# zyansheep/shadow

Measured on AMD Instinct MI355X. Metric: APSP routing build (s) @10k nodes; packets routed/sec per sim round, lower is better.
Workload: dtype u64+f32; 1 GPU; C3 APSP routing build: 10k-node undirected ring+chords graph, mean degree 8, latency U[1,100] ms (integer us), loss 0 w.p. 0.8 else U(0,0.02); all nodes used; source rows sharded across ranks (each rank keeps its row block; the optional RCCL all-gather of the blocks is timed separately in apsp_detail.allgather_ms); nodes=10000, arcs=79996, parallelism=rows1

## Files before the change

### shadow_amd/csrc/sg_internal.h

```cpp
#pragma once

#include <hip/hip_runtime.h>

#include <cstdint>
#include <cstdio>
#include <new>
#include <stdexcept>
#include <string>
#include <atomic>
#include <deque>
#include <memory>
#include <vector>

#include "../../include/shadow_gpu.h"

namespace sg {

struct Error : std::runtime_error {
  int32_t code;
  uint32_t row, col;
  Error(int32_t c, const std::string& m, uint32_t r = 0, uint32_t k = 0)
      : std::runtime_error(m), code(c), row(r), col(k) {}
};

// ... 315 lines not shown

constexpr int SSSP_DIAG_WORDS = 16;
constexpr int SSSP_POP_CLASSES = 6;
constexpr int SSSP_POP_WORDS = 3 * SSSP_POP_CLASSES + 2;
struct SsspLdsLaunch {
  const uint32_t* d_used = nullptr;
  uint32_t n_used = 0, row_begin = 0, row_end = 0;
  bool ident = false;
  uint64_t* out_lat = nullptr;
  float* out_loss = nullptr;
  uint32_t* sat_row = nullptr;
  uint32_t delta = 0;
  unsigned long long* work = nullptr;
  unsigned long long* diag = nullptr;
  unsigned long long* pops = nullptr;
  const uint32_t* blk_rows = nullptr;
  uint32_t n_blk = 0;
  const uint32_t* ub_row = nullptr;
  const uint32_t* ub_w = nullptr;
  const uint32_t* plan_ctl = nullptr;
  int plan_ph = 0;
  uint32_t* plan_ctr = nullptr;
  uint32_t* done = nullptr;
  const SsspChainDesc* chain = nullptr;
};
void launch_sssp_lds(sg_ctx* ctx, const sg_net* net, const SsspLdsLaunch& l);

void ensure_csc(sg_ctx* ctx, sg_net* net);
void ensure_links(sg_ctx* ctx, sg_net* net);
std::string node_name(const sg_net* net, uint32_t idx);
void launch_zero2(sg_ctx* ctx, uint32_t* a, uint32_t na, uint32_t* b, uint32_t nb);

constexpr int WORK_SHARDS = 64;
void shortest_paths_slab(sg_ctx* ctx, sg_net* net, const uint32_t* d_used, uint32_t n_used, uint32_t row_begin,
                         uint32_t row_end, uint64_t* out_lat, float* out_loss);
void run_wide(sg_ctx* ctx, sg_net* net, const uint32_t* d_used, uint32_t n_used, const std::vector<uint32_t>& rows,
              uint32_t out_row0, uint64_t* out_lat, float* out_loss);

struct SsspDevPlan {
  int n_phase = 0;
  uint32_t* list = nullptr;
  uint32_t* ub_row = nullptr;
  uint32_t* ub_w = nullptr;
  uint32_t* ctl = nullptr;
  uint32_t* ctr = nullptr;
  const SsspChainDesc* chain = nullptr;
  bool landmarks = false;
  unsigned rows_grid = 0;
  bool bounds_deferred = false;
  const uint32_t* rel = nullptr;
  const uint8_t* phase_of = nullptr;
};
constexpr int SSSP_PHASES_MAX = 6;
SsspDevPlan sssp_device_plan(sg_ctx* ctx, sg_net* net, const uint32_t* d_used, uint32_t n_used, uint32_t row_begin,
                             uint32_t row_end, int n_phase, int kb, bool exact, int hops, uint32_t n_land,
                             uint32_t* zero_rows = nullptr, uint32_t* zero_rows2 = nullptr, bool chain = false,
                             bool chain_exact = false, bool defer_bounds = false);
void sssp_plan_bounds_side(sg_ctx* ctx, const sg_net* net, const SsspDevPlan& p, const uint32_t* d_used,
                           uint32_t row_begin, uint32_t row_end, int kb, bool exact, int hops);
const SsspChainDesc* sssp_plain_rel(sg_ctx* ctx, const sg_net* net, const uint32_t* d_used, uint32_t row_begin,
                                    uint32_t row_end, uint32_t* zero_rows, uint32_t* claim, uint32_t* zero_ctr,
                                    bool chain_exact);
void sssp_landmark_bounds(sg_ctx* ctx, const SsspDevPlan& p, uint32_t n_used, uint32_t row_begin,
                          const uint64_t* out_lat, const uint32_t* sat_row, int kb);

}
// ... 1 lines not shown
```

### shadow_amd/csrc/sg_routing.hip

```cpp
#include <algorithm>
#include <cstring>
#include <string>
#include <vector>

#include "sg_device.h"
#include "sg_internal.h"
#include "sg_knobs.h"

namespace sg {

__global__ void k_self_check(const uint32_t* __restrict__ used, uint32_t n_used,
                             const uint32_t* __restrict__ self_cnt,
                             unsigned long long* __restrict__ first) {
  for (uint32_t j = blockIdx.x * blockDim.x + threadIdx.x; j < n_used; j += gridDim.x * blockDim.x) {
    uint32_t c = self_cnt[used[j]];
    if (c != 1) atomicMin(first, ((unsigned long long)j << 1) | (c > 1 ? 1ull : 0ull));
  }
}

__global__ void __launch_bounds__(1024) k_build_finish(const uint32_t* __restrict__ sat, uint32_t rows,
                                                       const uint32_t* __restrict__ used, uint32_t n_used,
                                                       const uint32_t* __restrict__ self_cnt, uint32_t* __restrict__ ret,
                                                       int count_flags) {
  constexpr int G = 8;
// ... 288 lines not shown
  bool chain;
  bool overlap;
};
static LdsKnobs lds_knobs(const sg_ctx* ctx, const sg_net* net, uint32_t n_used, uint32_t rows) {
  LdsKnobs k;
  k.delta = (uint32_t)std::min(4294967295.0, std::max(1.0, knob_double("SG_APSP_DELTA", 4294967295.0)));
  k.diag = knob_int("SG_SSSP_DIAG", 0) != 0;
  const int seeds_env = knob_int("SG_SSSP_SEEDS", 1);
  const int flag_env = knob_int("SG_SSSP_FLAGGED", -1);
  const bool few_rows = rows < 6u * (uint32_t)std::max(1, ctx->n_cu);
  k.flagged = seeds_env != 0 && (flag_env == 1 || (flag_env < 0 && rows < n_used && !few_rows));
  k.phased = !k.flagged && seeds_env != 0 && (seeds_env == 2 || rows >= 8u * (uint32_t)ctx->n_cu);
  const bool chain = !knob_off("SG_SSSP_CHAIN") && !net->directed && !k.flagged;
  const uint32_t per_cu = rows / std::max(1, ctx->n_cu);
  k.n_phase = knob_int("SG_SSSP_PHASES", per_cu >= 16 && !chain ? 3 : 2, 2, SSSP_PHASES_MAX);
  k.kb = knob_int("SG_SSSP_BOUNDS", 2, 1, SSSP_KB_MAX);
  k.exact = knob_int("SG_SSSP_EXACT", 1) != 0 && n_used == net->n_nodes;
  k.hops = knob_int("SG_SSSP_HOPS", 3, 1, 3);
  const int land_env = knob_int("SG_SSSP_LANDMARKS", 0);
  k.n_land = net->directed || land_env <= 0 ? 0u : (uint32_t)land_env;
  k.chain = chain;
  k.overlap = build_fused();
  return k;
}

static void print_sssp_diag(sg_ctx* ctx, const sg_net* net, const unsigned long long* diag, uint32_t n_diag,
                            uint32_t delta) {
  constexpr int DW = SSSP_DIAG_WORDS;
  std::vector<unsigned long long> h((size_t)n_diag * DW);
  copy_to_host(ctx, h.data(), diag, h.size() * 8);
  double a[DW] = {};
  double setup = 0;
  double cn[2] = {0, 0}, cs[2] = {0, 0}, cq[2] = {0, 0};
  for (uint32_t r = 0; r < n_diag; r++) {
    for (int k = 0; k < DW; k++) a[k] += (double)h[(size_t)r * DW + k];
    const unsigned long long w3 = h[(size_t)r * DW + 3];
    setup += (double)(w3 >> 24);
    a[3] -= (double)(w3 >> 22 << 22);
    if (h[(size_t)r * DW] == 0) continue;
    const int c = (int)((w3 >> 22) & 1);
    cn[c] += 1;
    cs[c] += (double)(w3 >> 24);
    cq[c] += (double)h[(size_t)r * DW];
  }
  for (int c = 0; c < 2; c++)
    fprintf(stderr, "[sssp] %s rows: %.0f, mean setup %.0f cyc, mean search %.0f cyc\n", c ? "chained" : "unchained",
            cn[c], cs[c] / std::max(1.0, cn[c]), cq[c] / std::max(1.0, cn[c]));
  fprintf(stderr, "[sssp] mean setup (init + bound rows) %.0f cyc of the search\n", setup / n_diag);
  fprintf(stderr, "[sssp] setup parts: bound-row listing and load issue %.0f, LDS pass %.0f, barrier %.0f, first load "
          "round %.0f, later rounds and closing barrier %.0f cyc\n", a[9] / n_diag, a[8] / n_diag, a[10] / n_diag,
          a[11] / n_diag, a[12] / n_diag);
  fprintf(stderr, "[sssp] per-wave cycles summed over a row's 16 waves: claim+wait %.0f, pop %.0f, steps %.0f "
          "(per pop: %.0f, %.0f)\n", a[5] / n_diag, a[6] / n_diag, a[7] / n_diag, a[6] / std::max(1.0, a[2]),
          a[7] / std::max(1.0, a[2]));
  fprintf(stderr, "[sssp] delta %u ns, %u rows: mean search %.0f cyc, output %.0f cyc, %.1f wave pops, %.1f buckets, "
          "%.0f relaxations (%.2f x arcs)\n", delta, n_diag, a[0] / n_diag, a[1] / n_diag, a[2] / n_diag,
          a[3] / n_diag, a[4] / n_diag, a[4] / n_diag / std::max(1u, net->n_arcs));
}

static void shortest_paths_lds(sg_ctx* ctx, sg_net* net, const uint32_t* d_used, uint32_t n_used, uint32_t row_begin,
                               uint32_t row_end, uint64_t* out_lat, float* out_loss) {
  hipStream_t st = ctx->stream;
  const uint32_t rows = row_end - row_begin;
  const LdsKnobs k = lds_knobs(ctx, net, n_used, rows);
  *(volatile uint32_t*)(ctx->apsp_ret + 4) = 0u;
  bool told = false;
  struct SideDrain {
    sg_ctx* c;
    ~SideDrain() {
      if (c->side_busy) (void)hipStreamSynchronize(c->side_stream);
      c->side_busy = false;
    }
  } side_drain{ctx};
  uint32_t* sat = ctx->r_flags.get<uint32_t>(2 * (size_t)rows);
  uint32_t* claim = k.chain ? sat + rows : nullptr;
  constexpr int WORK_WORDS = WORK_SHARDS + 4 + SSSP_POP_WORDS;
  unsigned long long* work = ctx->count_work ? ctx->r_work.get<unsigned long long>(WORK_WORDS) : nullptr;
  if (work) SG_HIP(hipMemsetAsync(work, 0, WORK_WORDS * 8, st));
  unsigned long long pops_seen[SSSP_POP_WORDS] = {};
  auto diag_pops = [&](const char* what, int ph) {
    if (!work || !k.diag) return;
    unsigned long long c[SSSP_POP_WORDS];
    copy_to_host(ctx, c, work + WORK_SHARDS + 4, sizeof(c));
    static const char* const cls[SSSP_POP_CLASSES] = {"0", "1", "2", "3-4", "5-8", ">8"};
    for (int i = 0; i < SSSP_POP_CLASSES; i++) {
      const unsigned long long p = c[3 * i] - pops_seen[3 * i], a = c[3 * i + 1] - pops_seen[3 * i + 1],
                               cy = c[3 * i + 2] - pops_seen[3 * i + 2];
      fprintf(stderr, "[sssp] %s %d pops of S %s: %llu pops, %llu arcs, %llu step cycles (%.0f per pop)\n", what, ph,
              cls[i], p, a, cy, (double)cy / (double)std::max(1ull, p));
    }
    for (int i = 0; i < SSSP_POP_WORDS; i++) pops_seen[i] = c[i];
  };
  unsigned long long chained_seen[2] = {0, 0};
  unsigned long long phase_chained[SSSP_PHASES_MAX] = {};
  auto diag_chained = [&](const char* what, int ph) {
    if (!work) return;
    unsigned long long c[2];
    copy_to_host(ctx, c, work + WORK_SHARDS, 16);
    phase_chained[ph] = c[0] - chained_seen[0];
    if (k.diag)
      fprintf(stderr, "[sssp] %s %d: %llu chained rows, %llu with exact seeds\n", what, ph, c[0] - chained_seen[0],
              c[1] - chained_seen[1]);
    chained_seen[0] = c[0];
    chained_seen[1] = c[1];
  };
  auto publish_phases = [&](const SsspDevPlan& plan) {
    if (!work) return;
    uint32_t h[2 * SSSP_PHASES_MAX];
    copy_to_host(ctx, h, plan.ctl, sizeof(h));
// ... 82 lines not shown
      l.chain = sssp_plain_rel(ctx, net, d_used, row_begin, row_end, sat, claim, l.plan_ctr,
                               knob_int("SG_SSSP_EXACT", 1) != 0);
    } else {
      flush_used(ctx);
      launch_zero2(ctx, sat, rows, l.plan_ctr, 2u);
    }
    {
      TimedLaunch tl(ctx, "sssp", 0.0);
      launch_sssp_lds(ctx, net, l);
    }
    diag_chained("launch", 0);
    diag_pops("launch", 0);
  }
  if (diag) print_sssp_diag(ctx, net, diag, n_diag, k.delta);
  std::vector<uint32_t> wide_rows = finish_rows(ctx, sat, row_begin, rows, told);
  ctx->side_busy = false;
  if (work) {
    unsigned long long w[WORK_WORDS];
    timer_add_work(ctx, "sssp", read_work(ctx, work, w, WORK_WORDS - WORK_SHARDS));
    if (k.diag) {
      static const char* const cls[SSSP_POP_CLASSES] = {"0", "1", "2", "4", "8", "gt8"};
      const unsigned long long* pc = w + WORK_SHARDS + 4;
      for (int i = 0; i < SSSP_POP_CLASSES; i++) {
        char name[32];
        snprintf(name, sizeof(name), "sssp_pop_s%s", cls[i]);
        timer_set_counter(ctx, name, (double)pc[3 * i + 1], pc[3 * i]);
        snprintf(name, sizeof(name), "sssp_pop_s%s_cyc", cls[i]);
        timer_set_counter(ctx, name, (double)pc[3 * i + 2], pc[3 * i]);
      }
      timer_set_counter(ctx, "sssp_pops", (double)pc[3 * SSSP_POP_CLASSES], pc[SSSP_POP_WORDS - 1]);
    }
    timer_set_counter(ctx, "sssp_chained", (double)w[WORK_SHARDS], w[WORK_SHARDS + 1]);
    timer_set_counter(ctx, "sssp_ring_left", (double)w[WORK_SHARDS + 2], w[WORK_SHARDS + 3]);
    if (k.diag)
      fprintf(stderr, "[sssp] ring slots not empty at a row's end: %llu (%llu rows)\n", w[WORK_SHARDS + 2],
              w[WORK_SHARDS + 3]);
  }
  if (!wide_rows.empty()) run_wide(ctx, net, d_used, n_used, wide_rows, row_begin, out_lat, out_loss);
}

static void shortest_paths(sg_ctx* ctx, sg_net* net, const uint32_t* d_used, const uint32_t* h_used,
                           uint32_t n_used, uint32_t row_begin, uint32_t row_end, uint64_t* out_lat,
                           float* out_loss) {
  const bool per_source = knob_int("SG_APSP_LDS", 1) != 0;
  const bool dense_on = knob_int("SG_APSP_DENSE", 1) != 0;
  const int bucket_env = knob_int("SG_APSP_BUCKET", -1);
  const bool sparse = net->n_nodes && net->n_arcs <= 64ull * net->n_nodes;
  const bool arcs_ok = (uint64_t)net->n_arcs * 12 < (1ull << 31);
  const bool dense = per_source && dense_on && !sparse && sssp_dense_fits(net->n_nodes);
  const bool bucket = !dense && per_source && sparse && arcs_ok && bucket_env != 0 && sssp_bucket_fits(net->n_nodes) &&
                      (bucket_env == 1 || !sssp_lds_fits(net->n_nodes));
  const bool lds = !dense && !bucket && per_source && sparse && sssp_lds_fits(net->n_nodes) && arcs_ok;
  if (!lds) flush_used(ctx);
  if (dense)
    shortest_paths_dense(ctx, net, d_used, n_used, row_begin, row_end, out_lat, out_loss);
  else if (bucket)
    shortest_paths_bucket(ctx, net, d_used, n_used, row_begin, row_end, out_lat, out_loss);
  else if (lds)
    shortest_paths_lds(ctx, net, d_used, n_used, row_begin, row_end, out_lat, out_loss);
  else
    shortest_paths_slab(ctx, net, d_used, n_used, row_begin, row_end, out_lat, out_loss);
}


static void direct_paths(sg_ctx* ctx, sg_net* net, const uint32_t* d_used, const uint32_t* h_used,
                         uint32_t n_used, uint32_t row_begin, uint32_t row_end, uint64_t* out_lat,
// ... 293 lines not shown
```

### shadow_amd/csrc/sg_sssp.hip

```cpp
#include <algorithm>
#include <cstdlib>
#include <type_traits>

#include "sg_device.h"
#include "sg_internal.h"
#include "sg_knobs.h"

namespace sg {

constexpr int SSSP_THREADS = 1024;
constexpr int SSSP_WAVES = SSSP_THREADS / 64;
constexpr int SSSP_K = 4;
constexpr int SSSP_KB = SSSP_KB_MAX;
constexpr size_t SSSP_STATIC_LDS = 4 * (8 + SSSP_WAVES) + 16 + SSSP_WAVES * 64 * SSSP_K + 512 + 4 * (3 * SSSP_KB + 1) + 16;

constexpr size_t LDS_PER_CU = 160 * 1024;

constexpr uint64_t FKEY_INF = ((uint64_t)LAT32_SAT << 32) | ((uint64_t)0x3F800000u << 1);
__device__ __forceinline__ uint32_t fkey_lat(uint64_t k) { return (uint32_t)(k >> 32); }
__device__ __forceinline__ uint32_t fkey_loss_bits(uint64_t k) { return ((uint32_t)k >> 1) & 0x7FFFFFFFu; }
__device__ __forceinline__ uint64_t frelax(uint64_t ku, uint32_t edge_lat, float edge_om) {
  const uint32_t lat = __builtin_elementwise_add_sat(fkey_lat(ku), edge_lat);
  const float loss = fold_loss(__uint_as_float(fkey_loss_bits(ku)), edge_om);
  return ((uint64_t)lat << 32) | (uint32_t)((__float_as_uint(loss) << 1) | 1u);
// ... 15 lines not shown
  const uint64_t lt = (1ull << lane) - 1;
  uint32_t tot = 0;
#pragma unroll
  for (int c = 0; c < NK; c++) tot += (uint32_t)__popcll(mq[c]);
  if (!tot) return;
  uint32_t b = 0;
  if (lane == 0) b = atomicAdd(tail, tot);
  b = __builtin_amdgcn_readfirstlane(b);
#pragma unroll
  for (int c = 0; c < NK; c++) {
    if ((mq[c] >> lane) & 1ull) ring[slot_of(b + (uint32_t)__popcll(mq[c] & lt))] = (uint16_t)v[c];
    b += (uint32_t)__popcll(mq[c]);
  }
}

size_t sssp_lds_bytes(uint32_t n) {
  return (size_t)n * 8 + (((size_t)n + 1) * 4 + 7) / 8 * 8 + (size_t)sssp_ring_cap(n) * 2;
}

constexpr int SSSP_SC1 = 16;
template <bool COUNT, int NT, int LA, int PART, bool FLAG = false>
__global__ void __launch_bounds__(NT)
    k_sssp_lds(const uint32_t* __restrict__ out_off, const uint32_t* __restrict__ out_arc, uint32_t n,
               uint32_t n_arcs, const uint32_t* __restrict__ used, uint32_t n_used, uint32_t row_begin,
               uint32_t out_row0, const uint32_t* __restrict__ self_edge, const uint64_t* __restrict__ e_lat,
               const float* __restrict__ e_loss, uint64_t* __restrict__ out_lat, float* __restrict__ out_loss,
               uint32_t* __restrict__ sat_row, uint32_t delta, int vec_out, unsigned long long* __restrict__ work,
               unsigned long long* __restrict__ diag, uint32_t claim, uint32_t idle_sleep,
               uint32_t lane_deg_max, const uint32_t* __restrict__ blk_rows,
               const uint32_t* __restrict__ ub_row, const uint32_t* __restrict__ ub_w,
               uint32_t* __restrict__ item_ctr, uint32_t n_items, uint32_t spin_max,
               const uint32_t* __restrict__ plan_ctl, int plan_ph, uint32_t* __restrict__ done,
               const SsspChainDesc* chain_desc, uint32_t* __restrict__ any_flag, int ident, uint32_t step_arcs,
               unsigned long long* __restrict__ popc) {
  constexpr int NW = NT / 64;
  constexpr int AUX = FLAG ? SSSP_SC1 : 0;
  if (FLAG || !item_ctr) chain_desc = nullptr;
  const bool chain_on = chain_desc != nullptr;
  auto chain_args = [&]() {
    const SsspChainDesc* d = chain_desc;
    asm volatile("" : "+s"(d));
    return d;
  };
  if (plan_ctl) {
    const uint32_t base = plan_ctl[2 * plan_ph];
    n_items = plan_ctl[2 * plan_ph + 1];
    blk_rows += base;
    if (ub_row) {
      ub_row += (size_t)base * SSSP_KB;
      ub_w += (size_t)base * SSSP_KB;
    }
  }
  extern __shared__ __align__(16) unsigned char smem[];
  const uint32_t cap = sssp_ring_cap(n);
  const RingMod slot_of{cap, (uint32_t)(0x100000000ull / cap)};
  unsigned long long* key = (unsigned long long*)smem;
  uint32_t* off = (uint32_t*)(key + n);
  uint16_t* ring = (uint16_t*)(smem + (size_t)n * 8 + (((size_t)n + 1) * 4 + 7) / 8 * 8);
  unsigned long long* s_popc = (unsigned long long*)(ring + cap);
  const bool pop_diag = COUNT && popc;
  __shared__ uint32_t ctl[8];
  constexpr int TAIL = 1;
  __shared__ unsigned long long hb;
  __shared__ uint8_t own[NW][64 * SSSP_K];
  __shared__ uint32_t red[NW];
  __shared__ unsigned long long sink[64];
  __shared__ uint32_t s_ub[SSSP_KB][3];
  __shared__ uint32_t s_nub;
  __shared__ uint32_t s_sat;
  if (FLAG && threadIdx.x == 0) s_sat = 0u;

  const int tid = threadIdx.x, lane = tid & 63, wv = tid >> 6;
  constexpr uint32_t OOB = 0x80000000u;
  {
    const __amdgpu_buffer_rsrc_t ro = __builtin_amdgcn_make_buffer_rsrc((void*)out_off, 0, (int)((n + 1) * 4u),
                                                                        0x00020000);
    constexpr int GO = 12;
    for (uint32_t v0 = tid; v0 <= n; v0 += GO * NT) {
      uint32_t to[GO];
#pragma unroll
      for (int g = 0; g < GO; g++) {
        const uint32_t v = v0 + g * NT;
        to[g] = __builtin_amdgcn_raw_buffer_load_b32(ro, v <= n ? v * 4u : OOB, 0, 0);
      }
#pragma unroll
      for (int g = 0; g < GO; g++)
        if (v0 + g * NT <= n) off[v0 + g * NT] = to[g];
    }
  }
  __shared__ uint32_t s_item;
  __shared__ uint32_t s_chain, s_cw, s_psat;
  auto next_listed = [&]() -> uint32_t {
    uint32_t* claim_w = chain_on ? chain_args()->claim : nullptr;
    for (;;) {
      const uint32_t b = atomicAdd(item_ctr, 1u);
// ... 63 lines not shown
      } else {
        __builtin_amdgcn_fence(__ATOMIC_RELEASE, "wavefront");
        __builtin_amdgcn_wave_barrier();
        __builtin_amdgcn_fence(__ATOMIC_ACQUIRE, "wavefront");
      }
      nb = (int)s_nub;
    }
    unsigned long long c_list = 0, c_init = 0, c_bar = 0, c_g0 = 0;
    auto lds_pass = [&]() {
      if (dg) c_list = clock64();
      if (chain) {
        const bool ex = (chain & 2u) != 0;
        for (uint32_t v = tid; v < n; v += NT) {
          const uint64_t kv = key[v];
          const uint64_t lw = (uint64_t)fkey_lat(kv) + chain_w;
          uint64_t nk = FKEY_INF;
          if (fkey_lat(kv) != LAT32_SAT && lw < LAT32_SAT - 1)
            nk = ex ? (lw << 32) | ((uint32_t)kv & ~1u) : ((lw + 1) << 32) | ((uint64_t)0x3F800000u << 1);
          key[v] = nk;
        }
        if (COUNT && tid == 0) {
          atomicAdd(&work[WORK_SHARDS], 1ull);
          if (ex) atomicAdd(&work[WORK_SHARDS + 1], 1ull);
        }
      } else {
        for (uint32_t v = tid; v < n; v += NT) key[v] = FKEY_INF;
      }
      if (tid < 8) ctl[tid] = 0;
      if (tid == 0) hb = 0;
      if (dg) c_init = clock64();
      __syncthreads();
      if (dg) c_bar = clock64();
    };
    if (!nb) {
      lds_pass();
    } else {
      constexpr int GC = 10;
      const __amdgpu_buffer_rsrc_t ru = __builtin_amdgcn_make_buffer_rsrc((void*)used, 0, (int)(n_used * 4u),
                                                                          0x00020000);
      int k = 0;
      uint32_t jb = 0;
      uint32_t ts = (uint32_t)tid;
      asm volatile("" : "+v"(ts));
#pragma unroll 1
      do {
        const uint32_t j0 = jb + ts;
        uint32_t vv[GC];
        uint64_t l[2][GC];
        uint32_t f[2][GC];
        bool on[2], exact[2];
        uint32_t sr[2];
#pragma unroll
        for (int u = 0; u < 2; u++) {
          on[u] = k + u < nb;
          sr[u] = on[u] ? __builtin_amdgcn_readfirstlane(s_ub[k + u][0]) : 0u;
          exact[u] = on[u] && __builtin_amdgcn_readfirstlane(s_ub[k + u][2]);
          const size_t rb = on[u] ? (size_t)(sr[u] - out_row0) * n_used : 0;
          const __amdgpu_buffer_rsrc_t rl =
              __builtin_amdgcn_make_buffer_rsrc((void*)(out_lat + rb), 0, (int)(on[u] ? n_used * 8u : 0u), 0x00020000);
          const __amdgpu_buffer_rsrc_t rf = __builtin_amdgcn_make_buffer_rsrc(
              (void*)(out_loss + rb), 0, (int)(exact[u] ? n_used * 4u : 0u), 0x00020000);
#pragma unroll
          for (int g = 0; g < GC; g++) {
            const uint32_t j = j0 + g * NT;
            const auto x = __builtin_amdgcn_raw_buffer_load_b64(rl, j < n_used ? j * 8u : OOB, 0, AUX);
            l[u][g] = ((uint64_t)x[1] << 32) | x[0];
            f[u][g] = __builtin_amdgcn_raw_buffer_load_b32(rf, j < n_used ? j * 4u : OOB, 0, AUX);
          }
        }
        if (!ident) {
#pragma unroll
          for (int g = 0; g < GC; g++) {
            const uint32_t j = j0 + g * NT;
            vv[g] = __builtin_amdgcn_raw_buffer_load_b32(ru, j < n_used ? j * 4u : OOB, 0, 0);
          }
        }
        if (k == 0 && jb == 0) lds_pass();
        uint32_t w[2];
#pragma unroll
        for (int u = 0; u < 2; u++) w[u] = on[u] ? __builtin_amdgcn_readfirstlane(s_ub[k + u][1]) : 0u;
#pragma unroll
        for (int g = 0; g < GC; g++) {
          const uint32_t j = j0 + g * NT;
          if (j >= n_used) continue;
          const uint32_t v = ident ? j : vv[g];
          const uint64_t k0 = key[v];
          uint64_t kv = k0;
#pragma unroll
          for (int u = 0; u < 2; u++) {
            const uint64_t ub = l[u][g] + w[u];
            if (!on[u] || ub < w[u]) continue;
            if (ub < LAT32_SAT - 1) kv = min(kv, ((ub + 1) << 32) | ((uint64_t)0x3F800000u << 1));
            if (exact[u] && ub < LAT32_SAT && j != sr[u])
              kv = min(kv, (ub << 32) | ((uint64_t)f[u][g] << 1));
          }
          if (kv != k0) key[v] = kv;
        }
        if (dg && !c_g0) c_g0 = clock64();
        jb += GC * NT;
        if (jb >= n_used) {
          jb = 0;
          k += 2;
        }
      } while (k < nb);
    }
    if (ub_row) __syncthreads();
    const unsigned long long c_setup = dg ? clock64() : 0;
    if (tid == 0) {
      key[src] = 1ull;
      ring[0] = (uint16_t)src;
      ctl[TAIL] = 1;
      s_psat = 0u;
    }
    uint32_t split = delta;
    const __amdgpu_buffer_rsrc_t arcs = __builtin_amdgcn_make_buffer_rsrc((void*)out_arc, 0, (int)(n_arcs * 12u),
                                                                          0x00020000);
    uint32_t n_rel = 0;
    const uint32_t max_adv = 4u * n + 64u;
    uint8_t* ow = own[wv];
    uint32_t spins = 0;
    constexpr int ABORT = 2;
    auto give_up = [&]() {
      if (lane == 0) {
        sat_row[row - row_begin] = 2u;
        *any_flag = 1u;
        if (atomicExch(&ctl[ABORT], 1u) == 0u && item_ctr) {
          __threadfence();
          if (atomicAdd(&item_ctr[1], 1u) == gridDim.x - 1) {
            const uint32_t c = __hip_atomic_load(&item_ctr[0], __ATOMIC_RELAXED, __HIP_MEMORY_SCOPE_AGENT);
            uint32_t* claim_w = chain_on ? chain_args()->claim : nullptr;
            for (uint32_t i = min(c, n_items); i < n_items; i++) {
              const uint32_t r = (blk_rows ? blk_rows[i] : row_begin + i) - row_begin;
              if (!claim_w || __hip_atomic_load(&claim_w[r], __ATOMIC_RELAXED, __HIP_MEMORY_SCOPE_AGENT) == 0u)
                sat_row[r] = 2u;
            }
          }
        }
      }
    };
    auto ld = [](uint32_t* p) { return __hip_atomic_load(p, __ATOMIC_RELAXED, __HIP_MEMORY_SCOPE_WORKGROUP); };
    auto offer_all = [&](auto nk, const bool* valid, const uint32_t* v, const uint64_t* cand, uint64_t* app) {
      constexpr int NK = decltype(nk)::value;
      uint64_t cd[NK], old[NK];
      bool okk[NK];
#pragma unroll
      for (int c = 0; c < NK; c++) {
        const bool ok = valid[c] && fkey_lat(cand[c]) != LAT32_SAT;
        okk[c] = ok;
        cd[c] = cand[c];
        old[c] = __hip_atomic_fetch_min(ok ? &key[v[c]] : &sink[lane], (unsigned long long)cd[c], __ATOMIC_RELAXED,
                                        __HIP_MEMORY_SCOPE_WORKGROUP);
      }
      __builtin_amdgcn_sched_barrier(0);
#pragma unroll
      for (int c = 0; c < NK; c++)
        app[c] = __builtin_amdgcn_ballot_w64(okk[c] && !((uint32_t)old[c] & 1u) && old[c] > cd[c] &&
                                             fkey_lat(cd[c]) < split);
    };
    __syncthreads();

    for (;;) {
      const unsigned long long tc0 = (COUNT && diag) ? clock64() : 0;
      uint32_t h = 0, k = 0;
      if (lane == 0) {
        for (;;) {
          const unsigned long long w = __hip_atomic_load(&hb, __ATOMIC_RELAXED, __HIP_MEMORY_SCOPE_WORKGROUP);
          const uint32_t hh = (uint32_t)(w >> 32), t = ld(&ctl[TAIL]);
          if (t == hh) break;
          const uint32_t kk = min(claim, t - hh);
          const unsigned long long nw = ((unsigned long long)(hh + kk) << 32) | ((w & 0xFFFFFFFFull) + 1);
          if (atomicCAS(&hb, w, nw) == w) {
            h = hh;
            k = kk;
            break;
          }
        }
      }
      h = __builtin_amdgcn_readfirstlane(h);
      k = __builtin_amdgcn_readfirstlane(k);
      if (__builtin_amdgcn_readfirstlane(ld(&ctl[ABORT]))) goto wave_exit;
      if (!k) {
        uint32_t q = 0;
        if (lane == 0) {
          const unsigned long long w = __hip_atomic_load(&hb, __ATOMIC_RELAXED, __HIP_MEMORY_SCOPE_WORKGROUP);
          __atomic_signal_fence(__ATOMIC_SEQ_CST);
          q = (w & 0xFFFFFFFFull) == 0 && (uint32_t)(w >> 32) == ld(&ctl[TAIL]);
        }
        if (!__builtin_amdgcn_readfirstlane(q)) {
          if (++spins > spin_max) {
            give_up();
            goto wave_exit;
          }
          for (uint32_t z = 0; z < idle_sleep; z++) __builtin_amdgcn_s_sleep(8);
// ... 1 lines not shown
          continue;
        }
        __syncthreads();
        if (ld(&ctl[ABORT])) goto wave_exit;
        if (split >= LAT32_SAT) break;
        uint32_t m = LAT32_SAT;
        for (uint32_t v = tid; v < n; v += NT) {
          const uint64_t kv = key[v];
          if (kv & 1ull) m = min(m, fkey_lat(kv));
        }
        for (int d = 32; d > 0; d >>= 1) m = min(m, (uint32_t)__shfl_xor(m, d));
        if (lane == 0) red[wv] = m;
        __syncthreads();
        m = red[0];
        for (int w = 1; w < NW; w++) m = min(m, red[w]);
        if (m == LAT32_SAT) break;
        if (++n_adv > max_adv) {
          give_up();
          goto wave_exit;
        }
        split = m + delta >= m ? min(m + delta, LAT32_SAT) : LAT32_SAT;
        for (uint32_t v0 = wv * 64; v0 < n; v0 += NT) {
          const uint32_t v = v0 + lane;
          uint64_t kv = v < n ? key[v] : 0ull;
          const bool q2 = (kv & 1ull) && fkey_lat(kv) < split;
          const uint64_t m2 = __ballot(q2);
          append_q<1>(&m2, &v, ring, &ctl[TAIL], slot_of, lane);
        }
        __syncthreads();
        continue;
      }
      if (COUNT) n_pops++;
      const unsigned long long tc1 = (COUNT && diag) ? clock64() : 0;
      const bool on = lane < (int)k;
      uint32_t u = 0, a0 = 0, a1 = 0;
      uint64_t ku = 0;
      bool stuck = false;
      if (on) {
        uint16_t* slot = &ring[slot_of(h + lane)];
        uint16_t x;
        uint32_t sp = 0;
        while ((x = __hip_atomic_load(slot, __ATOMIC_RELAXED, __HIP_MEMORY_SCOPE_WORKGROUP)) == RING_EMPTY &&
               ++sp < spin_max)
          __builtin_amdgcn_s_sleep(0);
        stuck = x == RING_EMPTY;
        __hip_atomic_store(slot, RING_EMPTY, __ATOMIC_RELAXED, __HIP_MEMORY_SCOPE_WORKGROUP);
        u = stuck ? src : x;
        a0 = off[u];
        a1 = off[u + 1];
        ku = __hip_atomic_fetch_and(&key[u], ~1ull, __ATOMIC_RELAXED, __HIP_MEMORY_SCOPE_WORKGROUP) & ~1ull;
      }
      if (__any(stuck)) {
        give_up();
        goto wave_exit;
      }
      const uint32_t deg = a1 - a0;
      const uint32_t deg_incl = wave_incl_sum(deg);
      const uint32_t T = __builtin_amdgcn_readlane(deg_incl, 63);
      const unsigned long long tc2 = (COUNT && (diag || pop_diag)) ? clock64() : 0;
      auto expand = [&](auto kx, uint32_t ea0, uint32_t edeg, uint32_t incl) {
        constexpr int KX = decltype(kx)::value;
        const uint32_t base = incl - edeg;
        const uint32_t T = __builtin_amdgcn_readlane(incl, 63);
        if (COUNT) n_rel += T;
        uint32_t carry = 0;
        for (uint32_t t0 = 0; t0 < T; t0 += 64 * KX) {
// ... 68 lines not shown
        }
      }
      if (lane == 0) atomicSub(&hb, 1ull);
      if (COUNT && (diag || pop_diag)) {
        const unsigned long long tc3 = clock64();
        if (diag) {
          cyc_claim += tc1 - tc0;
          cyc_pop += tc2 - tc1;
          cyc_steps += tc3 - tc2;
        }
        if (pop_diag && lane == 0) {
          const uint32_t S = (T + 63u) / 64u;
          const int cls = S <= 2u ? (int)S : S <= 4u ? 3 : S <= 8u ? 4 : 5;
          atomicAdd(&s_popc[3 * cls], 1ull);
          atomicAdd(&s_popc[3 * cls + 1], (unsigned long long)T);
          atomicAdd(&s_popc[3 * cls + 2], tc3 - tc2);
        }
      }
    }
    if (COUNT && lane == 0 && n_rel) atomicAdd(&work[bi & 63], (unsigned long long)n_rel);
    if (COUNT && diag && bi < 4096 && lane == 0) {
      if (n_rel) atomicAdd(&diag[bi * SSSP_DIAG_WORDS + 4], (unsigned long long)n_rel);
      if (n_pops) atomicAdd(&diag[bi * SSSP_DIAG_WORDS + 2], (unsigned long long)n_pops);
      atomicAdd(&diag[bi * SSSP_DIAG_WORDS + 5], cyc_claim);
      atomicAdd(&diag[bi * SSSP_DIAG_WORDS + 6], cyc_pop);
      atomicAdd(&diag[bi * SSSP_DIAG_WORDS + 7], cyc_steps);
    }
    const unsigned long long c_search = dg ? clock64() : 0;
    if (COUNT) {
      uint32_t left = 0;
      for (uint32_t i = tid; i < cap; i += NT) left += ring[i] != RING_EMPTY;
      if (left) atomicAdd(&work[WORK_SHARDS + 2], (unsigned long long)left);
      if (tid == 0) atomicAdd(&work[WORK_SHARDS + 3], 1ull);
    }

    __syncthreads();
    if (pop_diag) {
      if (tid < SSSP_POP_WORDS - 1 && s_popc[tid]) {
        atomicAdd(&popc[tid], s_popc[tid]);
        s_popc[tid] = 0ull;
      }
      if (lane == 0 && n_pops) atomicAdd(&popc[SSSP_POP_WORDS - 1], (unsigned long long)n_pops);
    }
    if (item_ctr && !chain_on) {
      if (wv == 0) {
        uint32_t ni = 0;
        if (lane == 0) s_item = ni = atomicAdd(item_ctr, 1u);
        if (!FLAG && ub_row) {
          ni = __builtin_amdgcn_readfirstlane(ni);
          if (ni < n_items) list_bounds(ni);
        }
      }
    } else if (item_ctr && wv == NW - 1) {
      uint32_t ll = (uint32_t)lane;
      asm volatile("" : "+v"(ll));
      const SsspChainDesc* cd = chain_args();
      uint32_t* claim_w = cd->claim;
      const uint32_t* rel = cd->rel;
      const uint8_t* phase_of = cd->phase_of;
      const uint32_t* list_pos = cd->pos;
      const uint32_t a0 = off[src], nd = min(off[src + 1] - a0, 64u);
      const bool in = ll < nd;
      const auto r = __builtin_amdgcn_raw_buffer_load_b96(arcs, in ? (a0 + ll) * 12u : OOB, 0, 0);
      const __amdgpu_buffer_rsrc_t rr = __builtin_amdgcn_make_buffer_rsrc((void*)rel, 0, (int)(n * 4u), 0x00020000);
      const uint32_t q = __builtin_amdgcn_raw_buffer_load_b32(rr, in ? r[0] * 4u : OOB, 0, 0);
      bool ok = in && q != ~0u;
// ... 127 lines not shown
        st_lat2(j, l0, l1);
        st_lat2(j + 2, l2, l3);
        st_loss4(j, f0, f1, f2, f3);
      }
    } else {
      for (uint32_t j = tid; j < n_used; j += NT) {
        uint64_t l;
        float f;
        entry(j, l, f);
        if constexpr (FLAG) {
          __builtin_amdgcn_raw_buffer_store_b64((uint32_t __attribute__((ext_vector_type(2)))){(uint32_t)l,
                                                                                              (uint32_t)(l >> 32)},
                                                wl, j * 8u, 0, SSSP_SC1);
          __builtin_amdgcn_raw_buffer_store_b32(__float_as_uint(f), wf, j * 4u, 0, SSSP_SC1);
        } else {
          out_lat[orow + j] = l;
          out_loss[orow + j] = f;
        }
      }
    }
    if (__any(sat) && lane == 0) {
      sat_row[row - row_begin] = 1u;
      *any_flag = 1u;
      if (FLAG) s_sat = 1u;
      if (chain_on) s_psat = 1u;
    }
    if (dg) {
      diag[bi * SSSP_DIAG_WORDS + 0] = c_search - c_start;
      diag[bi * SSSP_DIAG_WORDS + 1] = clock64() - c_search;
      diag[bi * SSSP_DIAG_WORDS + 3] = n_adv | ((unsigned long long)chain << 22) | ((c_setup - c_start) << 24);
      diag[bi * SSSP_DIAG_WORDS + 8] = c_init - c_list;
      diag[bi * SSSP_DIAG_WORDS + 9] = c_list - c_start;
      diag[bi * SSSP_DIAG_WORDS + 10] = c_bar - c_list;
      diag[bi * SSSP_DIAG_WORDS + 11] = c_g0 - c_bar;
      diag[bi * SSSP_DIAG_WORDS + 12] = c_setup - c_g0;
    }
    if constexpr (FLAG) {
      asm volatile("s_waitcnt vmcnt(0)" ::: "memory");
      __syncthreads();
      if (tid == 0) {
        const __amdgpu_buffer_rsrc_t rd = __builtin_amdgcn_make_buffer_rsrc((void*)done, 0, 0x7FFFFFFF, 0x00020000);
        __builtin_amdgcn_raw_buffer_store_b32(s_sat ? 2u : 1u, rd, (row - row_begin) * 4u, 0, SSSP_SC1);
        s_sat = 0u;
      }
    }
    __syncthreads();
  }
wave_exit:;
}

bool sssp_lds_fits(uint32_t n) {
  if (n == 0 || n >= RING_EMPTY) return false;
  return sssp_lds_bytes(n) + SSSP_STATIC_LDS <= LDS_PER_CU;
}

struct SsspKnobs {
  uint32_t claim;
  uint32_t idle_sleep;
  uint32_t lane_deg;
  bool persist;
  uint32_t spin_max;
  uint32_t step_arcs;
};
static SsspKnobs sssp_knobs() {
  SsspKnobs k;
  k.claim = (uint32_t)knob_int("SG_SSSP_CLAIM", 64, 1, 64);
  k.idle_sleep = (uint32_t)std::max(0, knob_int("SG_SSSP_SLEEP", 0));
  k.lane_deg = (uint32_t)std::max(0, knob_int("SG_SSSP_LANE_DEG", 64));
  k.persist = !knob_off("SG_SSSP_PERSIST");
  k.spin_max = sssp_spin_max();
  k.step_arcs = (uint32_t)std::max(0, knob_int("SG_SSSP_STEP_ARCS", 256));
  return k;
}

void launch_sssp_lds(sg_ctx* ctx, const sg_net* net, const SsspLdsLaunch& l) {
  const SsspKnobs k = sssp_knobs();
  const uint32_t n = net->n_nodes;
  size_t lds = sssp_lds_bytes(n);
  if (!sssp_lds_fits(n)) throw Error(SG_ERR_INVALID_ARG, "graph too large for the LDS-resident search");
  if ((uint64_t)net->n_arcs * 12 >= (1ull << 31)) throw Error(SG_ERR_INVALID_ARG, "too many arcs for 32-bit offsets");
  const int vec = l.n_used % 4 == 0 && ((uintptr_t)l.out_lat & 15) == 0 && ((uintptr_t)l.out_loss & 15) == 0;
  const uint32_t rows = l.blk_rows ? l.n_blk : l.row_end - l.row_begin;
  if (!rows) return;
  const bool persist = l.done || (k.persist && (rows > (uint32_t)ctx->n_cu || l.plan_ctl));
  uint32_t* item_ctr = nullptr;
  if (persist && l.plan_ctr) {
    item_ctr = l.plan_ctr;
  } else if (persist) {
    item_ctr = ctx->r_items.get<uint32_t>(2);
    SG_HIP(hipMemsetAsync(item_ctr, 0, 8, ctx->stream));
  }
  const uint32_t grid = persist ? (uint32_t)ctx->n_cu : rows;
  const SsspChainDesc* chain = persist && !l.done && !net->directed ? l.chain : nullptr;
  unsigned long long* pops = l.work ? l.pops : nullptr;
  if (pops && lds + SSSP_POP_WORDS * 8 + SSSP_STATIC_LDS > LDS_PER_CU) pops = nullptr;
  if (pops) lds += SSSP_POP_WORDS * 8;
  auto go = [&](auto kern) {
    SG_HIP(hipFuncSetAttribute((const void*)kern, hipFuncAttributeMaxDynamicSharedMemorySize,
                               (int)(LDS_PER_CU - SSSP_STATIC_LDS)));
    hipLaunchKernelGGL(kern, dim3(grid), dim3(1024), lds, ctx->stream, net->out_off, net->out_arc, n, net->n_arcs,
                       l.d_used, l.n_used, l.row_begin, l.row_begin, net->self_edge, net->e_lat, net->e_loss,
                       l.out_lat, l.out_loss, l.sat_row, l.delta, vec, l.work, l.diag, k.claim, k.idle_sleep,
                       k.lane_deg, l.blk_rows, l.ub_row, l.ub_w, item_ctr, rows, k.spin_max, l.plan_ctl, l.plan_ph,
                       l.done, chain, ctx->apsp_ret + 4, (int)l.ident, k.step_arcs, pops);
  };
  if (l.done) {
    if (l.work) go(k_sssp_lds<true, 1024, 8, 0, true>);
    else if (ctx->in_fill) go(k_sssp_lds<false, 1024, 8, 1, true>);
    else go(k_sssp_lds<false, 1024, 8, 0, true>);
  } else if (l.work) {
    go(k_sssp_lds<true, 1024, 8, 0>);
  } else if (ctx->in_fill) {
    go(k_sssp_lds<false, 1024, 8, 1>);
  } else {
    go(k_sssp_lds<false, 1024, 8, 0>);
  }
  SG_CHECK_LAUNCH();
}


}
```

Measured before the change: 2.477 ms.

## Start chained SSSP rows immediately and merge bound-row seeds concurrently via CAS

For chained rows after the first item, the search now starts right after the LDS pass. Waves 1..15 stream the bound-row latency/loss seeds from global memory and merge them into the LDS keys with CAS loops, while wave 0 (and then all waves) begins popping. The aim is to hide the bound-row load and setup latency behind the search instead of paying it up front under a barrier. The cost is CAS contention on LDS keys, searches that start with weaker bounds (possibly more relaxations), and merges onto keys already marked dirty. It also adds diagnostic counters for the early path.

```diff
diff --git a/shadow_amd/csrc/sg_internal.h b/shadow_amd/csrc/sg_internal.h
--- a/shadow_amd/csrc/sg_internal.h
+++ b/shadow_amd/csrc/sg_internal.h
@@ -371,6 +371,7 @@
 void launch_zero2(sg_ctx* ctx, uint32_t* a, uint32_t na, uint32_t* b, uint32_t nb);
 
 constexpr int WORK_SHARDS = 64;
+constexpr int WORK_SSSP_EARLY = WORK_SHARDS + 4 + SSSP_POP_WORDS;
 void shortest_paths_slab(sg_ctx* ctx, sg_net* net, const uint32_t* d_used, uint32_t n_used, uint32_t row_begin,
                          uint32_t row_end, uint64_t* out_lat, float* out_loss);
 void run_wide(sg_ctx* ctx, sg_net* net, const uint32_t* d_used, uint32_t n_used, const std::vector<uint32_t>& rows,
diff --git a/shadow_amd/csrc/sg_routing.hip b/shadow_amd/csrc/sg_routing.hip
--- a/shadow_amd/csrc/sg_routing.hip
+++ b/shadow_amd/csrc/sg_routing.hip
@@ -344,9 +344,27 @@
   double a[DW] = {};
   double setup = 0;
   double cn[2] = {0, 0}, cs[2] = {0, 0}, cq[2] = {0, 0};
+  double en[2] = {0, 0}, e1[2] = {0, 0}, e4[2] = {0, 0}, e4n[2] = {0, 0}, ew[2] = {0, 0}, em = 0, ed = 0;
+  double parts_n = 0;
   for (uint32_t r = 0; r < n_diag; r++) {
-    for (int k = 0; k < DW; k++) a[k] += (double)h[(size_t)r * DW + k];
+    for (int k = 0; k < 13; k++) a[k] += (double)h[(size_t)r * DW + k];
     const unsigned long long w3 = h[(size_t)r * DW + 3];
+    if (h[(size_t)r * DW] != 0 && ((w3 >> 22) & 1)) {
+      const unsigned long long w13 = h[(size_t)r * DW + 13], w14 = h[(size_t)r * DW + 14], w15 = h[(size_t)r * DW + 15];
+      const int e = (int)((w15 >> 32) & 1);
+      en[e] += 1;
+      e1[e] += (double)(uint32_t)w14;
+      if ((uint32_t)w13) {
+        e4[e] += (double)(uint32_t)w13;
+        e4n[e] += 1;
+      }
+      ew[e] += (double)(w13 >> 32);
+      if (e) {
+        em += (double)(w14 >> 32);
+        ed += (double)(uint32_t)w15;
+      }
+    }
+    if (!((h[(size_t)r * DW + 15] >> 32) & 1)) parts_n += 1;
     setup += (double)(w3 >> 24);
     a[3] -= (double)(w3 >> 22 << 22);
     if (h[(size_t)r * DW] == 0) continue;
@@ -360,8 +378,14 @@
             cn[c], cs[c] / std::max(1.0, cn[c]), cq[c] / std::max(1.0, cn[c]));
   fprintf(stderr, "[sssp] mean setup (init + bound rows) %.0f cyc of the search\n", setup / n_diag);
   fprintf(stderr, "[sssp] setup parts: bound-row listing and load issue %.0f, LDS pass %.0f, barrier %.0f, first load "
-          "round %.0f, later rounds and closing barrier %.0f cyc\n", a[9] / n_diag, a[8] / n_diag, a[10] / n_diag,
-          a[11] / n_diag, a[12] / n_diag);
+          "round %.0f, later rounds and closing barrier %.0f cyc (%.0f rows)\n", a[9] / n_diag, a[8] / n_diag,
+          a[10] / n_diag, a[11] / std::max(1.0, parts_n), a[12] / std::max(1.0, parts_n), parts_n);
+  for (int e = 0; e < 2; e++)
+    fprintf(stderr, "[sssp] chained rows %s: %.0f, from the search's start: first claim %.0f cyc, fourth claim %.0f cyc "
+            "(%.0f rows), %.2f waves with a claim in the first 16k cyc\n", e ? "started under their loads" : "set up first",
+            en[e], e1[e] / std::max(1.0, en[e]), e4[e] / std::max(1.0, e4n[e]), e4n[e], ew[e] / std::max(1.0, en[e]));
+  fprintf(stderr, "[sssp] rows started under their loads: last wave merged %.0f cyc after the search's start, %.2f merges "
+          "onto dirty keys per row\n", em / std::max(1.0, en[1]), ed / std::max(1.0, en[1]));
   fprintf(stderr, "[sssp] per-wave cycles summed over a row's 16 waves: claim+wait %.0f, pop %.0f, steps %.0f "
           "(per pop: %.0f, %.0f)\n", a[5] / n_diag, a[6] / n_diag, a[7] / n_diag, a[6] / std::max(1.0, a[2]),
           a[7] / std::max(1.0, a[2]));
@@ -386,7 +410,7 @@
   } side_drain{ctx};
   uint32_t* sat = ctx->r_flags.get<uint32_t>(2 * (size_t)rows);
   uint32_t* claim = k.chain ? sat + rows : nullptr;
-  constexpr int WORK_WORDS = WORK_SHARDS + 4 + SSSP_POP_WORDS;
+  constexpr int WORK_WORDS = WORK_SSSP_EARLY + 2;
   unsigned long long* work = ctx->count_work ? ctx->r_work.get<unsigned long long>(WORK_WORDS) : nullptr;
   if (work) SG_HIP(hipMemsetAsync(work, 0, WORK_WORDS * 8, st));
   unsigned long long pops_seen[SSSP_POP_WORDS] = {};
@@ -535,6 +559,7 @@
     }
     timer_set_counter(ctx, "sssp_chained", (double)w[WORK_SHARDS], w[WORK_SHARDS + 1]);
     timer_set_counter(ctx, "sssp_ring_left", (double)w[WORK_SHARDS + 2], w[WORK_SHARDS + 3]);
+    timer_set_counter(ctx, "sssp_early", (double)w[WORK_SSSP_EARLY + 1], w[WORK_SSSP_EARLY]);
     if (k.diag)
       fprintf(stderr, "[sssp] ring slots not empty at a row's end: %llu (%llu rows)\n", w[WORK_SHARDS + 2],
               w[WORK_SHARDS + 3]);
diff --git a/shadow_amd/csrc/sg_sssp.hip b/shadow_amd/csrc/sg_sssp.hip
--- a/shadow_amd/csrc/sg_sssp.hip
+++ b/shadow_amd/csrc/sg_sssp.hip
@@ -71,7 +71,7 @@
                uint32_t* __restrict__ item_ctr, uint32_t n_items, uint32_t spin_max,
                const uint32_t* __restrict__ plan_ctl, int plan_ph, uint32_t* __restrict__ done,
                const SsspChainDesc* chain_desc, uint32_t* __restrict__ any_flag, int ident, uint32_t step_arcs,
-               unsigned long long* __restrict__ popc) {
+               unsigned long long* __restrict__ popc, int early_on) {
   constexpr int NW = NT / 64;
   constexpr int AUX = FLAG ? SSSP_SC1 : 0;
   if (FLAG || !item_ctr) chain_desc = nullptr;
@@ -100,6 +100,7 @@
   const bool pop_diag = COUNT && popc;
   __shared__ uint32_t ctl[8];
   constexpr int TAIL = 1;
+  constexpr int E_DIRTY = 0, E_T0 = 3, E_POPS = 4, E_WAVES = 5, E_T4 = 6, E_T1 = 7;
   __shared__ unsigned long long hb;
   __shared__ uint8_t own[NW][64 * SSSP_K];
   __shared__ uint32_t red[NW];
@@ -229,12 +230,59 @@
       __syncthreads();
       if (dg) c_bar = clock64();
     };
-    if (!nb) {
+    struct BoundPair {
+      bool on[2], exact[2];
+      uint32_t sr[2];
+    };
+    const __amdgpu_buffer_rsrc_t ru_set = __builtin_amdgcn_make_buffer_rsrc((void*)used, 0, (int)(n_used * 4u),
+                                                                            0x00020000);
+    auto bound_loads = [&](auto gc, int k, uint32_t j0, uint32_t stride, BoundPair& p, auto& l, auto& f, auto& vv) {
+      constexpr int GC = decltype(gc)::value;
+#pragma unroll
+      for (int u = 0; u < 2; u++) {
+        p.on[u] = k + u < nb;
+        p.sr[u] = p.on[u] ? __builtin_amdgcn_readfirstlane(s_ub[k + u][0]) : 0u;
+        p.exact[u] = p.on[u] && __builtin_amdgcn_readfirstlane(s_ub[k + u][2]);
+        const size_t rb = p.on[u] ? (size_t)(p.sr[u] - out_row0) * n_used : 0;
+        const __amdgpu_buffer_rsrc_t rl =
+            __builtin_amdgcn_make_buffer_rsrc((void*)(out_lat + rb), 0, (int)(p.on[u] ? n_used * 8u : 0u), 0x00020000);
+        const __amdgpu_buffer_rsrc_t rf = __builtin_amdgcn_make_buffer_rsrc(
+            (void*)(out_loss + rb), 0, (int)(p.exact[u] ? n_used * 4u : 0u), 0x00020000);
+#pragma unroll
+        for (int g = 0; g < GC; g++) {
+          const uint32_t j = j0 + g * stride;
+          const auto x = __builtin_amdgcn_raw_buffer_load_b64(rl, j < n_used ? j * 8u : OOB, 0, AUX);
+          l[u][g] = ((uint64_t)x[1] << 32) | x[0];
+          f[u][g] = __builtin_amdgcn_raw_buffer_load_b32(rf, j < n_used ? j * 4u : OOB, 0, AUX);
+        }
+      }
+      if (!ident) {
+#pragma unroll
+        for (int g = 0; g < GC; g++) {
+          const uint32_t j = j0 + g * stride;
+          vv[g] = __builtin_amdgcn_raw_buffer_load_b32(ru_set, j < n_used ? j * 4u : OOB, 0, 0);
+        }
+      }
+    };
+    auto bound_seed = [&](const BoundPair& p, const uint32_t* w, uint32_t j, uint64_t l0, uint64_t l1, uint32_t f0,
+                          uint32_t f1) {
+      uint64_t sd = ~0ull;
+#pragma unroll
+      for (int u = 0; u < 2; u++) {
+        const uint64_t ub = (u ? l1 : l0) + w[u];
+        if (!p.on[u] || ub < w[u]) continue;
+        if (ub < LAT32_SAT - 1) sd = min(sd, ((ub + 1) << 32) | ((uint64_t)0x3F800000u << 1));
+        if (p.exact[u] && ub < LAT32_SAT && j != p.sr[u])
+          sd = min(sd, (ub << 32) | ((uint64_t)(u ? f1 : f0) << 1));
+      }
+      return sd;
+    };
+    const bool early = !FLAG && early_on && chain && nb > 0 && it > 0;
+    if (!nb || early) {
       lds_pass();
+      if (COUNT && early && tid == 0) atomicAdd(&work[WORK_SSSP_EARLY], 1ull);
     } else {
       constexpr int GC = 10;
-      const __amdgpu_buffer_rsrc_t ru = __builtin_amdgcn_make_buffer_rsrc((void*)used, 0, (int)(n_used * 4u),
-                                                                          0x00020000);
       int k = 0;
       uint32_t jb = 0;
       uint32_t ts = (uint32_t)tid;
@@ -245,53 +293,19 @@
         uint32_t vv[GC];
         uint64_t l[2][GC];
         uint32_t f[2][GC];
-        bool on[2], exact[2];
-        uint32_t sr[2];
-#pragma unroll
-        for (int u = 0; u < 2; u++) {
-          on[u] = k + u < nb;
-          sr[u] = on[u] ? __builtin_amdgcn_readfirstlane(s_ub[k + u][0]) : 0u;
-          exact[u] = on[u] && __builtin_amdgcn_readfirstlane(s_ub[k + u][2]);
-          const size_t rb = on[u] ? (size_t)(sr[u] - out_row0) * n_used : 0;
-          const __amdgpu_buffer_rsrc_t rl =
-              __builtin_amdgcn_make_buffer_rsrc((void*)(out_lat + rb), 0, (int)(on[u] ? n_used * 8u : 0u), 0x00020000);
-          const __amdgpu_buffer_rsrc_t rf = __builtin_amdgcn_make_buffer_rsrc(
-              (void*)(out_loss + rb), 0, (int)(exact[u] ? n_used * 4u : 0u), 0x00020000);
-#pragma unroll
-          for (int g = 0; g < GC; g++) {
-            const uint32_t j = j0 + g * NT;
-            const auto x = __builtin_amdgcn_raw_buffer_load_b64(rl, j < n_used ? j * 8u : OOB, 0, AUX);
-            l[u][g] = ((uint64_t)x[1] << 32) | x[0];
-            f[u][g] = __builtin_amdgcn_raw_buffer_load_b32(rf, j < n_used ? j * 4u : OOB, 0, AUX);
-          }
-        }
-        if (!ident) {
-#pragma unroll
-          for (int g = 0; g < GC; g++) {
-            const uint32_t j = j0 + g * NT;
-            vv[g] = __builtin_amdgcn_raw_buffer_load_b32(ru, j < n_used ? j * 4u : OOB, 0, 0);
-          }
-        }
+        BoundPair p;
+        bound_loads(std::integral_constant<int, GC>(), k, j0, (uint32_t)NT, p, l, f, vv);
         if (k == 0 && jb == 0) lds_pass();
         uint32_t w[2];
 #pragma unroll
-        for (int u = 0; u < 2; u++) w[u] = on[u] ? __builtin_amdgcn_readfirstlane(s_ub[k + u][1]) : 0u;
+        for (int u = 0; u < 2; u++) w[u] = p.on[u] ? __builtin_amdgcn_readfirstlane(s_ub[k + u][1]) : 0u;
 #pragma unroll
         for (int g = 0; g < GC; g++) {
           const uint32_t j = j0 + g * NT;
           if (j >= n_used) continue;
           const uint32_t v = ident ? j : vv[g];
-          const uint64_t k0 = key[v];
-          uint64_t kv = k0;
-#pragma unroll
-          for (int u = 0; u < 2; u++) {
-            const uint64_t ub = l[u][g] + w[u];
-            if (!on[u] || ub < w[u]) continue;
-            if (ub < LAT32_SAT - 1) kv = min(kv, ((ub + 1) << 32) | ((uint64_t)0x3F800000u << 1));
-            if (exact[u] && ub < LAT32_SAT && j != sr[u])
-              kv = min(kv, (ub << 32) | ((uint64_t)f[u][g] << 1));
-          }
-          if (kv != k0) key[v] = kv;
+          const uint64_t sd = bound_seed(p, w, j, l[0][g], l[1][g], f[0][g], f[1][g]);
+          if (sd < key[v]) key[v] = sd;
         }
         if (dg && !c_g0) c_g0 = clock64();
         jb += GC * NT;
@@ -301,14 +315,16 @@
         }
       } while (k < nb);
     }
-    if (ub_row) __syncthreads();
+    if (ub_row && !early) __syncthreads();
     const unsigned long long c_setup = dg ? clock64() : 0;
     if (tid == 0) {
       key[src] = 1ull;
       ring[0] = (uint16_t)src;
       ctl[TAIL] = 1;
       s_psat = 0u;
-    }
+      if (COUNT && diag) ctl[E_T0] = (uint32_t)clock64();
+    }
+    if (COUNT && diag && lane == 0) red[wv] = 0u;
     uint32_t split = delta;
     const __amdgpu_buffer_rsrc_t arcs = __builtin_amdgcn_make_buffer_rsrc((void*)out_arc, 0, (int)(n_arcs * 12u),
                                                                           0x00020000);
@@ -356,6 +372,49 @@
     };
     __syncthreads();
 
+    if (early && wv != 0) {
+      constexpr int GE = 11;
+      constexpr uint32_t NM = NT - 64;
+      uint32_t ts = (uint32_t)tid - 64u;
+      asm volatile("" : "+v"(ts));
+      int k = 0;
+      uint32_t jb = 0;
+#pragma unroll 1
+      do {
+        const uint32_t j0 = jb + ts;
+        uint32_t vv[GE];
+        uint64_t l[2][GE];
+        uint32_t f[2][GE];
+        BoundPair p;
+        bound_loads(std::integral_constant<int, GE>(), k, j0, NM, p, l, f, vv);
+        uint32_t w[2];
+#pragma unroll
+        for (int u = 0; u < 2; u++) w[u] = p.on[u] ? __builtin_amdgcn_readfirstlane(s_ub[k + u][1]) : 0u;
+#pragma unroll
+        for (int g = 0; g < GE; g++) {
+          const uint32_t j = j0 + g * NM;
+          if (j >= n_used) continue;
+          const uint32_t v = ident ? j : vv[g];
+          const uint64_t sd = bound_seed(p, w, j, l[0][g], l[1][g], f[0][g], f[1][g]);
+          unsigned long long old = __hip_atomic_load(&key[v], __ATOMIC_RELAXED, __HIP_MEMORY_SCOPE_WORKGROUP);
+          while (sd < (old & ~1ull)) {
+            const unsigned long long prev = atomicCAS(&key[v], old, sd | (old & 1ull));
+            if (prev == old) {
+              if (COUNT && (old & 1ull)) atomicAdd(&ctl[E_DIRTY], 1u);
+              break;
+            }
+            old = prev;
+          }
+        }
+        jb += GE * NM;
+        if (jb >= n_used) {
+          jb = 0;
+          k += 2;
+        }
+      } while (k < nb);
+      if (COUNT && diag && lane == 0) red[wv] = (uint32_t)clock64() - ctl[E_T0];
+    }
+
     for (;;) {
       const unsigned long long tc0 = (COUNT && diag) ? clock64() : 0;
       uint32_t h = 0, k = 0;
@@ -423,6 +482,12 @@
       }
       if (COUNT) n_pops++;
       const unsigned long long tc1 = (COUNT && diag) ? clock64() : 0;
+      if (COUNT && diag && lane == 0) {
+        const uint32_t dt = (uint32_t)tc1 - ctl[E_T0], np = atomicAdd(&ctl[E_POPS], 1u);
+        if (np == 0u) ctl[E_T1] = dt;
+        if (np == 3u) ctl[E_T4] = dt;
+        if (dt < 16384u) atomicOr(&ctl[E_WAVES], 1u << wv);
+      }
       const bool on = lane < (int)k;
       uint32_t u = 0, a0 = 0, a1 = 0;
       uint64_t ku = 0;
@@ -557,6 +622,7 @@
       for (uint32_t i = tid; i < cap; i += NT) left += ring[i] != RING_EMPTY;
       if (left) atomicAdd(&work[WORK_SHARDS + 2], (unsigned long long)left);
       if (tid == 0) atomicAdd(&work[WORK_SHARDS + 3], 1ull);
+      if (tid == 0 && early && ctl[E_DIRTY]) atomicAdd(&work[WORK_SSSP_EARLY + 1], (unsigned long long)ctl[E_DIRTY]);
     }
 
     __syncthreads();
@@ -750,8 +816,13 @@
       diag[bi * SSSP_DIAG_WORDS + 8] = c_init - c_list;
       diag[bi * SSSP_DIAG_WORDS + 9] = c_list - c_start;
       diag[bi * SSSP_DIAG_WORDS + 10] = c_bar - c_list;
-      diag[bi * SSSP_DIAG_WORDS + 11] = c_g0 - c_bar;
-      diag[bi * SSSP_DIAG_WORDS + 12] = c_setup - c_g0;
+      diag[bi * SSSP_DIAG_WORDS + 11] = early ? 0ull : c_g0 - c_bar;
+      diag[bi * SSSP_DIAG_WORDS + 12] = early ? 0ull : c_setup - c_g0;
+      uint32_t last_merge = 0;
+      for (int w = 1; w < NW; w++) last_merge = max(last_merge, red[w]);
+      diag[bi * SSSP_DIAG_WORDS + 13] = ctl[E_T4] | ((unsigned long long)__popc(ctl[E_WAVES]) << 32);
+      diag[bi * SSSP_DIAG_WORDS + 14] = ctl[E_T1] | ((unsigned long long)(early ? last_merge : 0u) << 32);
+      diag[bi * SSSP_DIAG_WORDS + 15] = ctl[E_DIRTY] | ((unsigned long long)early << 32);
     }
     if constexpr (FLAG) {
       asm volatile("s_waitcnt vmcnt(0)" ::: "memory");
@@ -779,6 +850,7 @@
   bool persist;
   uint32_t spin_max;
   uint32_t step_arcs;
+  bool early;
 };
 static SsspKnobs sssp_knobs() {
   SsspKnobs k;
@@ -788,6 +860,7 @@
   k.persist = !knob_off("SG_SSSP_PERSIST");
   k.spin_max = sssp_spin_max();
   k.step_arcs = (uint32_t)std::max(0, knob_int("SG_SSSP_STEP_ARCS", 256));
+  k.early = knob_int("SG_SSSP_EARLY", 1) != 0;
   return k;
 }
 
@@ -820,7 +893,7 @@
                        l.d_used, l.n_used, l.row_begin, l.row_begin, net->self_edge, net->e_lat, net->e_loss,
                        l.out_lat, l.out_loss, l.sat_row, l.delta, vec, l.work, l.diag, k.claim, k.idle_sleep,
                        k.lane_deg, l.blk_rows, l.ub_row, l.ub_w, item_ctr, rows, k.spin_max, l.plan_ctl, l.plan_ph,
-                       l.done, chain, ctx->apsp_ret + 4, (int)l.ident, k.step_arcs, pops);
+                       l.done, chain, ctx->apsp_ret + 4, (int)l.ident, k.step_arcs, pops, (int)k.early);
   };
   if (l.done) {
     if (l.work) go(k_sssp_lds<true, 1024, 8, 0, true>);
```

New measurement: 2.413 ms (median of 6 runs). 2.6% less time.
